# HongwenZhang/DaNet-DensePose2SMPL

Hardware: AMD Instinct MI355X
Metric: images/sec fwd+bwd HRNet-W48+SMPL+IUV 256x256 bs32/GPU (higher is better)
Workload: dtype bf16; 1 GPU; full DaNet train step (HRNet-W48 + global and part-wise IUV heads + regressor nets + SMPL LBS (2 forward + 1 backward; the 2 label-side forwards belong to the untimed batch prologue) + IUV render + losses, fwd+bwd+Adam), 256x256, 32 img/GPU; convs bf16 MFMA fp32-acc, LBS/raster/losses fp32; global_batch=32, parallelism=dp1

## Files before the change

### danet-densepose2smpl_amd/_lib.py

```python
import ctypes
import os

_HERE = os.path.dirname(os.path.abspath(__file__))
LIB_PATH = os.environ.get('DANET_LIB') or os.path.join(_HERE, 'csrc', 'libdanet_hip.so')
_lib = None

c_f = ctypes.c_void_p
c_i = ctypes.c_int
c_sz = ctypes.c_size_t
c_fl = ctypes.c_float

_SIGNATURES = {
    'danet_version': (c_i, []),
    'danet_last_error': (ctypes.c_char_p, []),
    'danet_smpl_lbs_debug': (c_i, [c_f]),
    'danet_smpl_lbs_ctx_floats': (c_sz, [c_i]),
    'danet_smpl_lbs_fwd_ws_floats': (c_sz, [c_i, c_i, c_i]),
    'danet_smpl_lbs_bwd_ws_floats': (c_sz, [c_i, c_i, c_i]),
    'danet_smpl_lbs_ticket_words': (c_sz, [c_i]),
    'danet_smpl_lbs_forward': (c_i, [c_f, c_f, c_i] + [c_f] * 9 + [c_i] * 4 + [c_f] * 5 + [c_sz, c_f, c_f]),
    'danet_smpl_lbs_backward': (c_i, [c_f, c_f, c_i] + [c_f] * 7 + [c_i] * 4 + [c_f] * 7 + [c_sz, c_f, c_i, c_f]),
    'danet_smpl_lbs_backward_fused_ok': (c_i, [c_i, c_i, c_i]),
    'danet_iuv_raster_ws_bytes': (c_sz, [c_i, c_i, c_i]),
    'danet_iuv_raster_forward': (c_i, [c_f, c_f, c_i, c_i, c_f, c_i, c_f, c_f, c_i, c_fl, c_fl, c_i, c_f, c_f, c_f, c_f, c_sz, c_f]),
# ... 13 lines not shown
    'danet_conv_f32m_forward': (c_i, [c_f, c_f, c_f, c_f] + [c_i] * 15 + [c_f]),
    'danet_conv_f32m_wgrad_ws_floats': (c_sz, [c_i] * 15),
    'danet_conv_f32m_wgrad': (c_i, [c_f, c_f, c_f, c_f] + [c_i] * 15 + [c_f]),
    'danet_conv3x3_debug': (None, [c_f]),
    'danet_conv3x3_stream_plan': (c_i, [c_i] * 6),
    'danet_conv_stem_ok': (c_i, [c_i] * 13),
    'danet_conv_stem_forward': (c_i, [c_f, c_f, c_f] + [c_i] * 7 + [c_f, c_f]),
    'danet_conv_stem_dgrad_ok': (c_i, [c_i] * 13),
    'danet_conv_stem_dgrad': (c_i, [c_f, c_f, c_f] + [c_i] * 7 + [c_f] * 5),
    'danet_conv3x3a_ok': (c_i, [c_i] * 11),
    'danet_conv3x3a': (c_i, [c_f, c_f, c_f] + [c_i] * 4 + [c_f] * 5 + [c_i, c_f, c_f]),
    'danet_conv3x3_stream_table_bytes': (c_sz, []),
    'danet_conv3x3_stream_tables': (c_i, [c_f, c_sz]),
    'danet_conv_pack_weights_batched': (c_i, [c_f, c_i, ctypes.c_long, ctypes.c_long, c_f]),
    'danet_conv_pack_job_bricks': (ctypes.c_long, [c_i] * 7),
    'danet_conv_forward_multi_ok': (c_i, [c_f, c_i]),
    'danet_conv_forward_multi_kernel': (c_i, [c_f, c_i]),
    'danet_conv_forward_multi': (c_i, [c_f, c_i, c_f]),
    'danet_conv_forward_multi_epi_ok': (c_i, [c_f, c_i]),
    'danet_conv_forward_multi_epi_kernel': (c_i, [c_f, c_i]),
    'danet_conv_forward_multi_epi': (c_i, [c_f, c_i, c_f]),
    'danet_conv_stem_forward_epi': (c_i, [c_f, c_f, c_f, c_f] + [c_i] * 8 + [c_f]),
    'danet_conv3x3a_forward_epi': (c_i, [c_f] * 5 + [c_i] * 4 + [c_f]),
    'danet_conv_bn_forward_multi_ok': (c_i, [c_f, c_i, c_f, c_f]),
    'danet_conv_bn_forward_multi': (c_i, [c_f, c_i, c_f, c_fl, c_fl, c_f, c_f, c_f]),
    'danet_conv_forward_kernel': (c_i, [c_i] * 15),
    'danet_conv_forward': (c_i, [c_f] * 4 + [c_i] * 16 + [c_f] * 6 + [c_i, c_f]),
    'danet_conv_wgrad_rows_ok': (c_i, [c_i] * 13),
    'danet_conv_wgrad_rows_ws_floats': (c_sz, [c_i] * 8),
    'danet_conv_wgrad_rows': (c_i, [c_f] * 4 + [c_sz] + [c_i] * 12 + [c_fl, c_f]),
    'danet_conv_wgrad3x3_ok': (c_i, [c_i] * 10),
    'danet_conv_wgrad3x3_pair_ok': (c_i, [c_i] * 11),
    'danet_conv_wgrad3x3_ws_floats': (c_sz, [c_i] * 7),
    'danet_conv_wgrad_multi_ws_floats': (c_sz, [c_f, c_i]),
    'danet_conv_wgrad_multi_ws_zero_from': (c_sz, [c_f, c_i]),
    'danet_conv_wgrad_multi': (c_i, [c_f, c_i, c_f, c_sz, c_fl, c_f]),
    'danet_conv_wgrad3x3_multi_ws_floats': (c_sz, [c_f, c_i]),
    'danet_conv_wgrad3x3_multi': (c_i, [c_f, c_i, c_f, c_sz, c_fl, c_f]),
    'danet_conv_wgrad3x3_kernel_id': (c_i, [c_i] * 7),
    'danet_conv_wgrad3x3': (c_i, [c_f] * 4 + [c_sz] + [c_i] * 7 + [c_fl, c_i, c_f]),
    'danet_conv_wgrad_ws_floats': (c_sz, [c_i] * 4),
    'danet_conv_wgrad_ws_floats_for': (c_sz, [c_i] * 13),
    'danet_conv_wgrad': (c_i, [c_f] * 4 + [c_sz] + [c_i] * 13 + [c_fl, c_i, c_f]),
    'danet_bn_forward': (c_i, [c_f, c_f, c_f, ctypes.c_int64, c_i] + [c_f] * 6 + [c_i, c_fl, c_fl, c_i, c_i, c_f, c_f]),
    'danet_bn_ws_floats': (c_sz, [c_i]),
    'danet_knob': (ctypes.c_long, [c_i, ctypes.c_long]),
    'danet_bn_acc_bytes': (c_i, []),
    'danet_channel_sum': (c_i, [c_f, ctypes.c_int64, c_i, c_f, c_i, c_i, c_f]),
    'danet_bn_forward_multi': (c_i, [c_f, c_i, c_fl, c_fl, c_f]),
    'danet_bn_backward_multi': (c_i, [c_f, c_i, c_f]),
    'danet_bn_backward_onepass_ok': (c_i, [c_f, c_i, c_i]),
    'danet_bn_backward_onepass_bar_words': (c_i, []),
    'danet_bn_backward_onepass': (c_i, [c_f, c_i, c_f, c_i, c_f]),
    'danet_bn_backward': (c_i, [c_f, c_f, c_f, ctypes.c_int64, c_i, c_f, c_f, c_i, c_f, c_f, c_f, c_f, c_i, c_i, c_f, c_f, c_f]),
    'danet_sum_relu_forward': (c_i, [ctypes.POINTER(ctypes.c_void_p), ctypes.POINTER(c_i), c_i, c_i, c_i, c_i, c_i, c_i, c_f, c_f]),
    'danet_sum_relu_backward': (c_i, [c_f, c_f, c_i, c_i, c_i, c_i, c_i, c_i, c_f, c_f]),
    'danet_sum_relu_backward_all': (c_i, [c_f, c_f] + [c_i] * 5 + [c_f] * 5),
    'danet_sum_relu_forward_multi': (c_i, [c_f, c_i, c_f]),
    'danet_sum_relu_backward_all_multi': (c_i, [c_f, c_i, c_f]),
    'danet_maxpool3x3s2_forward': (c_i, [c_f, c_f, c_f, c_i, c_i, c_i, c_i, c_f]),
    'danet_maxpool3x3s2_backward': (c_i, [c_f, c_f, c_f, c_i, c_i, c_i, c_i, c_f]),
    'danet_stn_gather_forward': (c_i, [c_f, c_f] + [c_i] * 8 + [c_f, c_f]),
    'danet_stn_gather_backward': (c_i, [c_f, c_f] + [c_i] * 8 + [c_f, c_f]),
    'danet_part_clean_forward': (c_i, [c_f, c_f, c_i, c_i, c_i, c_i, c_f, c_f]),
    'danet_part_clean_backward': (c_i, [c_f, c_f, c_f, c_i, c_i, c_i, c_i, c_f, c_f]),
    'danet_part_loss_forward': (c_i, [c_f] * 5 + [c_i] * 5 + [c_f, c_f]),
# ... 219 lines not shown
```

### danet-densepose2smpl_amd/csrc/conv_wgrad3x3.hip

```cpp
#include <cstdlib>
#include "common.h"
#include "conv_common.h"

namespace {

using namespace danet_conv;

constexpr int TH = 4, TW = 8;
constexpr int halo_h(int st) { return st * (TH - 1) + 3; }
constexpr int halo_w(int st) { return st * (TW - 1) + 3; }

struct Wg3P {
    const bf16_t* x; const bf16_t* dy; float* part;
    float* direct;
    int B, H, W, Cin, Cout, groups, Cin_g, Cout_g;
    int IH, IW;
    int tiles_h, tiles_w, msplit;
    long nchunks;
    long x_bytes, dy_bytes;
};

typedef __attribute__((ext_vector_type(2))) unsigned v2u;

__device__ inline v2u tr_read(unsigned lds_byte_addr) {
    v2u r;
    asm volatile("ds_read_b64_tr_b16 %0, %1" : "=v"(r) : "v"(lds_byte_addr) : "memory");
    return r;
}

template <int CT, int NI, int ST, int SM = 0>
__device__ __forceinline__ void wgrad3x3_body(const Wg3P& p, const int bx, const int by, const int bz)
{
    constexpr bool PAIR = SM != 0;
    constexpr int OS = SM ? SM : 4;
    constexpr int PHW = ST * (OS - 1) + 3;
    constexpr int IMH = SM ? TH / OS : 1, IMW = SM ? TW / OS : 1;
    constexpr int HH = SM ? IMH * PHW : halo_h(ST), HW = SM ? IMW * PHW : halo_w(ST);
    constexpr int HALF = SM ? (4 / OS) * PHW : ST * 4;
    constexpr int BCO = CT * 16, BCI = NI * 16;
    constexpr int PXY = BCO * 2, PXX = BCI * 2;
    extern __shared__ __attribute__((aligned(16))) unsigned char smem[];
    constexpr int YB = TH * TW * PXY, XB = HH * HW * PXX, BUF = YB + XB;

    const int t = threadIdx.x, lane = t & 63, wave = t >> 6;
    const int li = lane & 15, lg = lane >> 4;
    const int nci = (p.Cin_g + BCI - 1) / BCI;
    const int cib = by % nci, cob = by / nci;
    const int g = bz;
    const int co0 = cob * BCO, ci0 = cib * BCI;
    const bf16_t* const dyg = p.dy + (size_t)g * p.Cout_g + co0;
    const bf16_t* const xg = p.x + (size_t)g * p.Cin_g + ci0;

    constexpr int NPAIR = 9 * NI;
    constexpr int MAXP = (NPAIR + 3) / 4;
    f32x4 acc[MAXP][CT];
    unsigned boff[MAXP];
#pragma unroll
    for (int pi = 0; pi < MAXP; ++pi) {
#pragma unroll
        for (int ct = 0; ct < CT; ++ct) acc[pi][ct] = f32x4{0.f, 0.f, 0.f, 0.f};
        const int pair = min(wave + 4 * pi, NPAIR - 1);
        const int tap = pair / NI, ni = pair - tap * NI;
        const int r = tap / 3, s = tap - r * 3;
        const int hrow = SM ? (lg / OS) * PHW + ST * (lg % OS) + r : ST * lg + r;
        const int hcol = SM ? ((li >> 2) / OS) * PHW + ST * ((li >> 2) % OS) + s : ST * (li >> 2) + s;
        boff[pi] = (unsigned)((hrow * HW + hcol) * PXX + (ni * 16 + 4 * (li & 3)) * 2);
    }
    const unsigned aoff = (unsigned)((lg * TW + (li >> 2)) * PXY + (4 * (li & 3)) * 2);

    const int nchunks = (int)p.nchunks;
    const int per = (nchunks + p.msplit - 1) / p.msplit;
    const int c_begin = bx * per, c_end = min(nchunks, c_begin + per);

    constexpr int NPY = TH * TW * (BCO / 8), NPX = HH * HW * (BCI / 8);
    constexpr int NRY = (NPY + 255) / 256, NRX = (NPX + 255) / 256;
    constexpr int OOB = 0x7fffffff;
    const __amdgpu_buffer_rsrc_t yr = __builtin_amdgcn_make_buffer_rsrc(const_cast<bf16_t*>(dyg), 0, (int)p.dy_bytes, 0x00020000);
    const __amdgpu_buffer_rsrc_t xr = __builtin_amdgcn_make_buffer_rsrc(const_cast<bf16_t*>(xg), 0, (int)p.x_bytes, 0x00020000);
    int yrel[NRY], xrel[NRX], xhy[NRX], xhx[NRX];
#pragma unroll
    for (int u = 0; u < NRY; ++u) {
        const int pc = t + u * 256;
        const int c8 = pc % (BCO / 8), q = pc / (BCO / 8);
        const int ty = q / TW, tx = q % TW;
        const int ypix = SM ? ((ty / OS) * IMW + tx / OS) * (OS * OS) + (ty % OS) * OS + tx % OS : ty * p.W + tx;
        yrel[u] = (pc < NPY && co0 + c8 * 8 < p.Cout_g) ? (ypix * p.Cout + c8 * 8) * 2 : OOB;
    }
#pragma unroll
    for (int u = 0; u < NRX; ++u) {
        const int pc = t + u * 256;
        const int c8 = pc % (BCI / 8), q = pc / (BCI / 8);
        const bool live = pc < NPX && ci0 + c8 * 8 < p.Cin_g;
        if (PAIR) {
            const int hq = q / HW, img = (hq / PHW) * IMW + (q % HW) / PHW, hy = hq % PHW - 1, hc = (q % HW) % PHW - 1;
            const bool inside = live && (unsigned)hy < (unsigned)(OS * ST) && (unsigned)hc < (unsigned)(OS * ST);
            xrel[u] = ((img * (OS * OS * ST * ST) + hy * (OS * ST) + hc) * p.Cin + c8 * 8) * 2;
            xhy[u] = inside ? 1 : -100000;
            xhx[u] = 1;
        } else {
            xrel[u] = (((q / HW - 1) * p.IW + q % HW - 1) * p.Cin + c8 * 8) * 2;
            xhy[u] = live ? q / HW : -100000;
            xhx[u] = q % HW;
        }
    }
    int f_tw = c_begin % p.tiles_w, f_th = (c_begin / p.tiles_w) % p.tiles_h, f_b = c_begin / (p.tiles_w * p.tiles_h);
    uint4 ystage[NRY], xstage[NRX];

    auto fetch = [&]() {
        const int oh0 = f_th * TH, ow0 = f_tw * TW;
        const int pix0 = (f_b * p.H + oh0) * p.W + ow0;
        const int by = pix0 * p.Cout * 2, bx = ((f_b * p.IH + ST * oh0) * p.IW + ST * ow0) * p.Cin * 2;
#pragma unroll
        for (int u = 0; u < NRY; ++u)
            ystage[u] = __builtin_bit_cast(uint4, __builtin_amdgcn_raw_buffer_load_b128(yr, yrel[u] != OOB ? by + yrel[u] : OOB, 0, 0));
#pragma unroll
        for (int u = 0; u < NRX; ++u) {
            const bool ok = PAIR ? xhy[u] > 0
                                 : ((unsigned)(ST * oh0 - 1 + xhy[u]) < (unsigned)p.IH && (unsigned)(ST * ow0 - 1 + xhx[u]) < (unsigned)p.IW);
            xstage[u] = __builtin_bit_cast(uint4, __builtin_amdgcn_raw_buffer_load_b128(xr, ok ? bx + xrel[u] : OOB, 0, 0));
        }
        if (++f_tw == p.tiles_w) { f_tw = 0; if (++f_th == p.tiles_h) { f_th = 0; ++f_b; } }
    };
    auto commit = [&](int buf) {
        unsigned char* base = smem + buf * BUF;
#pragma unroll
        for (int u = 0; u < NRY; ++u)
            if (t + u * 256 < NPY) *reinterpret_cast<uint4*>(base + (size_t)(t + u * 256) * 16) = ystage[u];
#pragma unroll
        for (int u = 0; u < NRX; ++u)
            if (t + u * 256 < NPX) *reinterpret_cast<uint4*>(base + (size_t)(NPY + t + u * 256) * 16) = xstage[u];
    };

    if (c_begin < c_end) fetch();
    int buf = 0;
    for (int ch = c_begin; ch < c_end; ++ch) {
        commit(buf);
        __syncthreads();
        if (ch + 1 < c_end) fetch();
        const unsigned ybase = (unsigned)(buf * BUF), xbase = ybase + YB;
        v2u alo[CT], ahi[CT], blo[MAXP], bhi[MAXP];
#pragma unroll
        for (int ct = 0; ct < CT; ++ct) {
            alo[ct] = tr_read(ybase + aoff + ct * 32);
            ahi[ct] = tr_read(ybase + aoff + ct * 32 + 4 * PXY);
        }
#pragma unroll
        for (int pi = 0; pi < MAXP; ++pi) {
            blo[pi] = tr_read(xbase + boff[pi]);
            bhi[pi] = tr_read(xbase + boff[pi] + HALF * PXX);
        }
        asm volatile("s_waitcnt lgkmcnt(0)" ::: "memory");
        __builtin_amdgcn_sched_barrier(0);
        bf16x8 a[CT];
#pragma unroll
        for (int ct = 0; ct < CT; ++ct) {
            const uint4 raw = {alo[ct].x, alo[ct].y, ahi[ct].x, ahi[ct].y};
            a[ct] = __builtin_bit_cast(bf16x8, raw);
        }
#pragma unroll
        for (int pi = 0; pi < MAXP; ++pi) {
            const uint4 raw = {blo[pi].x, blo[pi].y, bhi[pi].x, bhi[pi].y};
            const bf16x8 bq = __builtin_bit_cast(bf16x8, raw);
#pragma unroll
            for (int ct = 0; ct < CT; ++ct)
                acc[pi][ct] = __builtin_amdgcn_mfma_f32_16x16x32_bf16(a[ct], bq, acc[pi][ct], 0, 0, 0);
        }
        buf ^= 1;
    }
    const int gsz = 9 * p.Cout_g * p.Cin_g;
    if (p.direct) {
        float* const dw = p.direct + (size_t)g * gsz;
#pragma unroll
        for (int pi = 0; pi < MAXP; ++pi) {
            const int pair = wave + 4 * pi;
            const int tap = pair / NI, ni = pair - tap * NI;
            const int cin = ci0 + ni * 16 + li;
            if (pair >= NPAIR || cin >= p.Cin_g) continue;
#pragma unroll
            for (int ct = 0; ct < CT; ++ct)
#pragma unroll
                for (int r = 0; r < 4; ++r) {
                    const int cout = co0 + ct * 16 + lg * 4 + r;
                    if (cout < p.Cout_g) dw[((size_t)cout * p.Cin_g + cin) * 9 + tap] = acc[pi][ct][r];
                }
        }
        return;
    }
    float* dst = p.part + ((size_t)bx * p.groups + g) * gsz;
#pragma unroll
    for (int pi = 0; pi < MAXP; ++pi) {
        const int pair = wave + 4 * pi;
        const int tap = pair / NI, ni = pair - tap * NI;
        const int cin = ci0 + ni * 16 + li;
        if (pair >= NPAIR || cin >= p.Cin_g) continue;
        float* row = dst + ((tap * p.Cout_g + co0 + lg * 4) * p.Cin_g + cin);
#pragma unroll
        for (int ct = 0; ct < CT; ++ct)
#pragma unroll
            for (int r = 0; r < 4; ++r)
                if (co0 + ct * 16 + lg * 4 + r < p.Cout_g) row[(ct * 16 + r) * p.Cin_g] = acc[pi][ct][r];
    }
}

template <int CT, int NI, int ST>
__global__ __launch_bounds__(256) void conv_wgrad3x3_kernel(Wg3P p)
{
    wgrad3x3_body<CT, NI, ST>(p, blockIdx.x, blockIdx.y, blockIdx.z);
}

constexpr int NPM = 20;
struct Wg3Multi { Wg3P p[NPM]; int start[NPM + 1]; int nyb[NPM]; int n; int xcd; };

template <int CT, int NI, int ST, int SM = 0>
__global__ __launch_bounds__(256) void conv_wgrad3x3_multi_kernel(Wg3Multi mp)
{
    int vb = (int)blockIdx.x;
    if (mp.xcd) {
        const int G = (int)gridDim.x, q = G >> 3, r = G & 7;
        const int x = vb & 7, slot = vb >> 3;
        vb = x * q + (x < r ? x : r) + slot;
    }
    int i = 0;
    while (i + 1 < mp.n && vb >= mp.start[i + 1]) ++i;
    const int l = vb - mp.start[i];
    const Wg3P& p = mp.p[i];
    const int bx = l % p.msplit, rest = l / p.msplit;
    wgrad3x3_body<CT, NI, ST, SM>(p, bx, rest % mp.nyb[i], rest / mp.nyb[i]);
}

struct Red3Multi { const float* part[NPM]; float* dw[NPM]; int G[NPM], Cout_g[NPM], Cin_g[NPM], msplit[NPM]; long start[NPM + 1]; int n; float beta; };

__global__ __launch_bounds__(256) void wgrad3x3_reduce_multi_kernel(Red3Multi rp)
{
    const long gidx = (long)blockIdx.x * 256 + threadIdx.x;
    if (gidx >= rp.start[rp.n]) return;
    int i = 0;
    while (i + 1 < rp.n && gidx >= rp.start[i + 1]) ++i;
    const long idx = gidx - rp.start[i], total = rp.start[i + 1] - rp.start[i];
    const float* part = rp.part[i];
    float s = 0.f;
    int sp = 0;
    for (; sp + 4 <= rp.msplit[i]; sp += 4) {
        const float v0 = part[(size_t)sp * total + idx], v1 = part[(size_t)(sp + 1) * total + idx];
        const float v2 = part[(size_t)(sp + 2) * total + idx], v3 = part[(size_t)(sp + 3) * total + idx];
        s += (v0 + v1) + (v2 + v3);
    }
    for (; sp < rp.msplit[i]; ++sp) s += part[(size_t)sp * total + idx];
    const int Cin_g = rp.Cin_g[i], Cout_g = rp.Cout_g[i];
    const int cin = (int)(idx % Cin_g);
    long rest = idx / Cin_g;
    const int cout = (int)(rest % Cout_g); rest /= Cout_g;
    const int tap = (int)(rest % 9), g = (int)(rest / 9);
    const size_t o = (((size_t)(g * Cout_g + cout)) * Cin_g + cin) * 9 + tap;
    float* dw = rp.dw[i];
    dw[o] = rp.beta != 0.f ? dw[o] * rp.beta + s : s;
}

__global__ __launch_bounds__(256) void wgrad3x3_reduce_kernel(const float* __restrict__ part, float* __restrict__ dw,
                                                               int G, int Cout_g, int Cin_g, int msplit, float beta)
{
    const long total = (long)G * Cout_g * Cin_g * 9;
    const long idx = (long)blockIdx.x * 256 + threadIdx.x;
    if (idx >= total) return;
    float s = 0.f;
    int sp = 0;
    for (; sp + 4 <= msplit; sp += 4) {
        const float v0 = part[(size_t)sp * total + idx], v1 = part[(size_t)(sp + 1) * total + idx];
        const float v2 = part[(size_t)(sp + 2) * total + idx], v3 = part[(size_t)(sp + 3) * total + idx];
        s += (v0 + v1) + (v2 + v3);
    }
    for (; sp < msplit; ++sp) s += part[(size_t)sp * total + idx];
    const int cin = (int)(idx % Cin_g);
    long rest = idx / Cin_g;
    const int cout = (int)(rest % Cout_g); rest /= Cout_g;
    const int tap = (int)(rest % 9), g = (int)(rest / 9);
    const size_t o = (((size_t)(g * Cout_g + cout)) * Cin_g + cin) * 9 + tap;
    dw[o] = beta != 0.f ? dw[o] * beta + s : s;
}

template <int CT, int NI, int ST>
int launch3(const Wg3P& p, hipStream_t st) {
    const int nco = (p.Cout_g + CT * 16 - 1) / (CT * 16), nci = (p.Cin_g + NI * 16 - 1) / (NI * 16);
    const size_t lds = 2 * (size_t)(TH * TW * CT * 32 + halo_h(ST) * halo_w(ST) * NI * 32);
    hipLaunchKernelGGL((conv_wgrad3x3_kernel<CT, NI, ST>), dim3(p.msplit, nco * nci, p.groups), dim3(256), lds, st, p);
    return 0;
}

inline int tiles3(int c) { return c <= 16 ? 1 : (c <= 32 ? 2 : ((c % 48 == 0 || c <= 48) ? 3 : 4)); }

}

extern "C" int danet_conv_wgrad3x3_ok(int H, int W, int Cin, int Cout, int R, int S, int stride, int pad, int dil, int groups) {
    static const bool no_s2 = getenv("DANET_NO_WGRAD3_S2") != nullptr;
    if (!(R == 3 && S == 3 && (stride == 1 || (stride == 2 && !no_s2)) && pad == 1 && dil == 1)) return 0;
    if (H % stride != 0 || W % stride != 0) return 0;
    return (H / stride) % TH == 0 && (W / stride) % TW == 0 && (Cin / groups) % 8 == 0 && (Cout / groups) % 8 == 0;
}

extern "C" int danet_conv_wgrad3x3_pair_ok(int B, int H, int W, int Cin, int Cout, int R, int S, int stride, int pad, int dil, int groups) {
    static const bool off = getenv("DANET_NO_WGRAD3_PAIR") != nullptr;
    if (off || !(R == 3 && S == 3 && (stride == 1 || stride == 2) && pad == 1 && dil == 1 && H == W && B > 0 && groups > 0)) return 0;
    if (!((H == 4 * stride && B % 2 == 0) || (H == 2 * stride && B % 8 == 0))) return 0;
    if (Cin % groups != 0 || Cout % groups != 0) return 0;
    const int ci = Cin / groups, co = Cout / groups;
    if (ci % 8 != 0 || co % 8 != 0) return 0;
    return 1;
}
static inline int wg3_small(int B, int H, int W, int stride) {
    if (!(stride == 1 || stride == 2) || H != W) return 0;
    if (H == 4 * stride && B % 2 == 0) return 4;
    if (H == 2 * stride && B % 8 == 0) return 2;
    return 0;
}
static inline bool wg3_is_pair(int B, int H, int W, int stride) { return wg3_small(B, H, W, stride) != 0; }

static void plan3(int B, int H, int W, int Cin, int Cout, int groups, int* ct, int* ni, int* msplit) {
    const int Cout_g = Cout / groups, Cin_g = Cin / groups;
    *ct = tiles3(Cout_g); *ni = tiles3(Cin_g);
    if (*ct == 4) *ct = 2;
    if (*ni == 4) *ni = 2;
    const long other = (long)((Cout_g + *ct * 16 - 1) / (*ct * 16)) * ((Cin_g + *ni * 16 - 1) / (*ni * 16)) * groups;
    const long nchunks = (long)B * (H / TH) * (W / TW);
    long target = 256;
    if (const char* e = getenv("DANET_WGRAD3_BLOCKS")) target = atol(e);
    long ms = (target + other - 1) / other;
    if (ms > nchunks / 4) ms = nchunks / 4;
    if (ms < 1) ms = 1;
    *msplit = (int)ms;
}

extern "C" int danet_conv_wgrad3x3_kernel_id(int B, int H, int W, int Cin, int Cout, int groups, int stride) {
    int ct, ni, ms;
    plan3(B, H / stride, W / stride, Cin, Cout, groups, &ct, &ni, &ms);
    return ct * 10 + ni;
}

extern "C" size_t danet_conv_wgrad3x3_ws_floats(int B, int H, int W, int Cin, int Cout, int groups, int stride) {
    int ct, ni, ms;
    if (stride < 1) return 0;
    plan3(B, H / stride, W / stride, Cin, Cout, groups, &ct, &ni, &ms);
    return (size_t)ms * Cout * (Cin / groups) * 9;
}

extern "C" int danet_conv_wgrad3x3(const void* x, const void* dy, float* dw, float* ws, size_t ws_floats,
                                   int B, int H, int W, int Cin, int Cout, int groups, int stride, float beta, int phase, void* stream)
{
    DANET_ENTER();
    DANET_CHECK_ARG(x && dy && dw && ws && B > 0 && phase >= 0 && phase <= 2, "conv_wgrad3x3: bad arguments");
    DANET_CHECK_ARG(danet_conv_wgrad3x3_ok(H, W, Cin, Cout, 3, 3, stride, 1, 1, groups), "conv_wgrad3x3: unsupported shape");
    Wg3P p;
    p.x = (const bf16_t*)x; p.dy = (const bf16_t*)dy; p.part = ws; p.direct = nullptr;
    p.IH = H; p.IW = W; H /= stride; W /= stride;
    p.B = B; p.H = H; p.W = W; p.Cin = Cin; p.Cout = Cout; p.groups = groups;
    p.Cin_g = Cin / groups; p.Cout_g = Cout / groups;
    p.tiles_h = H / TH; p.tiles_w = W / TW;
    p.nchunks = (long)B * p.tiles_h * p.tiles_w;
    p.x_bytes = (long)B * p.IH * p.IW * Cin * 2; p.dy_bytes = (long)B * H * W * Cout * 2;
    DANET_CHECK_ARG(p.x_bytes < (1L << 31) && p.dy_bytes < (1L << 31), "conv_wgrad3x3: tensors of 2 GB or more are not supported");
    int ct, ni;
    plan3(B, H, W, Cin, Cout, groups, &ct, &ni, &p.msplit);
    if (ws_floats < (size_t)p.msplit * Cout * p.Cin_g * 9)
        return danet::fail(DANET_ERR_WORKSPACE, "conv_wgrad3x3: workspace too small");
    hipStream_t st = (hipStream_t)stream;
    if (phase != 2) {
#define W3(a, b) if (ct == a && ni == b) { if (stride == 1) launch3<a, b, 1>(p, st); else launch3<a, b, 2>(p, st); } else
        W3(1, 1) W3(1, 2) W3(1, 3) W3(2, 1) W3(2, 2) W3(2, 3) W3(3, 1) W3(3, 2) W3(3, 3)
        return danet::fail(DANET_ERR_ARG, "conv_wgrad3x3: no kernel for tiles %dx%d", ct, ni);
#undef W3
        DANET_CHECK_LAUNCH("conv_wgrad3x3_kernel");
    }
    if (phase == 1) return DANET_OK;
    const long total = (long)Cout * p.Cin_g * 9;
    hipLaunchKernelGGL(wgrad3x3_reduce_kernel, dim3(danet::cdiv(total, 256)), dim3(256), 0, st, ws, dw, groups, p.Cout_g,
                       p.Cin_g, p.msplit, beta);
    DANET_CHECK_LAUNCH("wgrad3x3_reduce_kernel");
    return DANET_OK;
}


struct Wg3Job { const void* x; const void* dy; float* dw; int B, H, W, Cin, Cout, groups, stride; };

static long multi_target_blocks() {
    if (const char* e = getenv("DANET_WGRAD3_MULTI_BLOCKS")) return atol(e);
    return 768;
}

static inline double wg3_weight(int Cout, int Cin_g) { const double p = (double)Cout * Cin_g; return p < 2304.0 ? 2304.0 : p; }
static void plan_multi(const Wg3Job* jobs, const int* idx, int cnt, int ct, int ni, int* msplit) {
    auto chunks_of = [](const Wg3Job& j) -> long {
        const int sm = wg3_small(j.B, j.H, j.W, j.stride);
        return sm ? (long)(j.B / (sm == 4 ? 2 : 8)) : (long)j.B * (j.H / j.stride / TH) * (j.W / j.stride / TW);
    };
    double tot = 0;
    for (int k = 0; k < cnt; ++k) {
        const Wg3Job& j = jobs[idx[k]];
        tot += (double)chunks_of(j) * wg3_weight(j.Cout, j.Cin / j.groups);
    }
    const long target = multi_target_blocks();
    for (int k = 0; k < cnt; ++k) {
        const Wg3Job& j = jobs[idx[k]];
        const int Cout_g = j.Cout / j.groups, Cin_g = j.Cin / j.groups;
        const long other = (long)((Cout_g + ct * 16 - 1) / (ct * 16)) * ((Cin_g + ni * 16 - 1) / (ni * 16)) * j.groups;
        const long nchunks = chunks_of(j);
        const double w = (double)nchunks * wg3_weight(j.Cout, Cin_g);
        long ms = (long)(target * (w / tot) / other + 0.5);
        if (ms > nchunks / 4) ms = nchunks / 4;
        if (ms < 1) ms = 1;
        msplit[k] = (int)ms;
    }
}

static int multi_foreach_launch(const Wg3Job* jobs, int n, float* ws, size_t ws_floats, float beta, hipStream_t st, size_t* need_out)
{
    size_t used = 0;
    bool done[4096];
    if (n > 4096) return danet::fail(DANET_ERR_ARG, "conv_wgrad3x3_multi: too many jobs (%d)", n);
    for (int i = 0; i < n; ++i) done[i] = false;
    for (int i = 0; i < n; ++i) {
        if (done[i]) continue;
        int ct, ni, dummy;
        const int stride = jobs[i].stride;
        const int sm = wg3_small(jobs[i].B, jobs[i].H, jobs[i].W, stride);
        const bool pair = sm != 0;
        plan3(jobs[i].B, jobs[i].H / stride, jobs[i].W / stride, jobs[i].Cin, jobs[i].Cout, jobs[i].groups, &ct, &ni, &dummy);
        static const int npm_env = getenv("DANET_WGRAD3_NPM") ? atoi(getenv("DANET_WGRAD3_NPM")) : 0;
        const int npm = npm_env > 0 && npm_env < NPM ? npm_env : NPM;
        int idx[NPM], cnt = 0;
        for (int k = i; k < n && cnt < npm; ++k) {
            if (done[k] || jobs[k].stride != stride || wg3_small(jobs[k].B, jobs[k].H, jobs[k].W, stride) != sm) continue;
            int c2, n2;
            plan3(jobs[k].B, jobs[k].H / stride, jobs[k].W / stride, jobs[k].Cin, jobs[k].Cout, jobs[k].groups, &c2, &n2, &dummy);
            if (c2 == ct && n2 == ni) { idx[cnt++] = k; done[k] = true; }
        }
        int msplit[NPM];
        plan_multi(jobs, idx, cnt, ct, ni, msplit);
        Wg3Multi mp; Red3Multi rp;
        static const bool xcd_order = getenv("DANET_WGRAD3_XCD") && atoi(getenv("DANET_WGRAD3_XCD")) != 0;
        mp.n = cnt; rp.n = cnt; rp.beta = beta; mp.xcd = xcd_order ? 1 : 0;
        mp.start[0] = 0; rp.start[0] = 0;
        for (int k = 0; k < cnt; ++k) {
            const Wg3Job& j = jobs[idx[k]];
            Wg3P& p = mp.p[k];
            static const bool no_direct = getenv("DANET_WGRAD3_NO_DIRECT") != nullptr;
            const bool direct = msplit[k] == 1 && beta == 0.f && !no_direct;
            p.x = (const bf16_t*)j.x; p.dy = (const bf16_t*)j.dy; p.part = (ws && !direct) ? ws + used : nullptr;
            p.direct = direct ? j.dw : nullptr;
            p.IH = j.H; p.IW = j.W;
            p.B = j.B; p.H = j.H / stride; p.W = j.W / stride; p.Cin = j.Cin; p.Cout = j.Cout; p.groups = j.groups;
            if (pair) { p.B = j.B / (sm == 4 ? 2 : 8); p.H = 4; p.W = 8; p.IH = 4 * stride; p.IW = 8 * stride; }
            p.Cin_g = j.Cin / j.groups; p.Cout_g = j.Cout / j.groups;
            p.tiles_h = p.H / TH; p.tiles_w = p.W / TW;
            p.nchunks = (long)p.B * p.tiles_h * p.tiles_w;
            p.x_bytes = (long)j.B * j.H * j.W * j.Cin * 2; p.dy_bytes = (long)j.B * (j.H / stride) * (j.W / stride) * j.Cout * 2;
            p.msplit = msplit[k];
            const int nyb = ((p.Cout_g + ct * 16 - 1) / (ct * 16)) * ((p.Cin_g + ni * 16 - 1) / (ni * 16));
            mp.nyb[k] = nyb;
            mp.start[k + 1] = mp.start[k] + msplit[k] * nyb * j.groups;
            const long total = (long)j.Cout * p.Cin_g * 9;
            rp.part[k] = p.part; rp.dw[k] = j.dw; rp.G[k] = j.groups; rp.Cout_g[k] = p.Cout_g; rp.Cin_g[k] = p.Cin_g; rp.msplit[k] = msplit[k];
            rp.start[k + 1] = rp.start[k] + (direct ? 0 : total);
            if (!direct || !ws) used += (size_t)msplit[k] * total;
            if (ws && !(p.x_bytes < (1L << 31) && p.dy_bytes < (1L << 31)))
                return danet::fail(DANET_ERR_ARG, "conv_wgrad3x3_multi: tensors of 2 GB or more are not supported");
        }
        if (!ws) continue;
        if (used > ws_floats) return danet::fail(DANET_ERR_WORKSPACE, "conv_wgrad3x3_multi: workspace too small");
        const int phw = stride * ((sm ? sm : 4) - 1) + 3;
        const size_t lds = 2 * (size_t)(TH * TW * ct * 32 + (sm ? (TH / sm) * phw * (TW / sm) * phw : halo_h(stride) * halo_w(stride)) * ni * 32);
        const dim3 grid((unsigned)mp.start[cnt]);
        if (pair) {
#define W3P(a, b) if (ct == a && ni == b) { \
            if (stride == 1 && sm == 4) hipLaunchKernelGGL((conv_wgrad3x3_multi_kernel<a, b, 1, 4>), grid, dim3(256), lds, st, mp); \
            else if (stride == 2 && sm == 4) hipLaunchKernelGGL((conv_wgrad3x3_multi_kernel<a, b, 2, 4>), grid, dim3(256), lds, st, mp); \
            else if (stride == 1) hipLaunchKernelGGL((conv_wgrad3x3_multi_kernel<a, b, 1, 2>), grid, dim3(256), lds, st, mp); \
            else hipLaunchKernelGGL((conv_wgrad3x3_multi_kernel<a, b, 2, 2>), grid, dim3(256), lds, st, mp); } else
            W3P(2, 2) W3P(2, 3) W3P(3, 2) W3P(3, 3) W3P(1, 1) W3P(1, 2) W3P(2, 1) W3P(1, 3) W3P(3, 1)
            return danet::fail(DANET_ERR_ARG, "conv_wgrad3x3_multi: no pair-mode kernel for tiles %dx%d", ct, ni);
#undef W3P
        } else
#define W3M(a, b) if (ct == a && ni == b) { \
            if (stride == 1) hipLaunchKernelGGL((conv_wgrad3x3_multi_kernel<a, b, 1>), grid, dim3(256), lds, st, mp); \
            else hipLaunchKernelGGL((conv_wgrad3x3_multi_kernel<a, b, 2>), grid, dim3(256), lds, st, mp); } else
        W3M(1, 1) W3M(1, 2) W3M(1, 3) W3M(2, 1) W3M(2, 2) W3M(2, 3) W3M(3, 1) W3M(3, 2) W3M(3, 3)
        return danet::fail(DANET_ERR_ARG, "conv_wgrad3x3_multi: no kernel for tiles %dx%d", ct, ni);
#undef W3M
        DANET_CHECK_LAUNCH("conv_wgrad3x3_multi_kernel");
        if (rp.start[cnt] > 0) {
            hipLaunchKernelGGL(wgrad3x3_reduce_multi_kernel, dim3((unsigned)danet::cdiv(rp.start[cnt], 256)), dim3(256), 0, st, rp);
            DANET_CHECK_LAUNCH("wgrad3x3_reduce_multi_kernel");
        }
    }
    if (need_out) *need_out = used;
    return DANET_OK;
}

extern "C" size_t danet_conv_wgrad3x3_multi_ws_floats(const void* jobs, int n)
{
    size_t need = 0;
    if (!jobs || n <= 0) return 0;
    multi_foreach_launch((const Wg3Job*)jobs, n, nullptr, 0, 0.f, nullptr, &need);
    return need;
}

// ... 13 lines not shown
```

### include/danet_hip.h

```cpp
#ifndef DANET_HIP_H
#define DANET_HIP_H

#include <stddef.h>
#include <stdint.h>

#ifdef __cplusplus
extern "C" {
#endif

#define DANET_OK 0
#define DANET_ERR_ARG (-1)
#define DANET_ERR_HIP (-2)
#define DANET_ERR_WORKSPACE (-3)

int danet_version(void);
const char* danet_last_error(void);

size_t danet_smpl_lbs_ctx_floats(int B);
size_t danet_smpl_lbs_fwd_ws_floats(int B, int V, int NE);
size_t danet_smpl_lbs_bwd_ws_floats(int B, int V, int NB);
size_t danet_smpl_lbs_ticket_words(int B);

int danet_smpl_lbs_forward(const float* betas, const float* rotmats, int B,
                           const float* v_template, const float* shapedirs, const float* posedirs,
// ... 161 lines not shown
       DANET_KNOB_PW = 10, DANET_KNOB_PW_WGRAD = 11, DANET_KNOB_STEM = 12, DANET_KNOB_STEM_DGRAD = 13, DANET_KNOB_C3A = 14,
       DANET_KNOB_BN_BLOCK_BYTES = 15, DANET_KNOB_C3S_BALANCE = 16, DANET_KNOB_C3S_TILE_COST = 17,
       DANET_KNOB_G3 = 18  };
long danet_knob(int id, long value);
int danet_conv3x3_stream_plan(int B, int H, int W, int Cin, int Cout, int nprob);
size_t danet_conv3x3_stream_table_bytes(void);
int danet_conv3x3_stream_tables(void* workspace, size_t bytes);
int danet_conv_stem_ok(int B, int H, int W, int Cin, int OH, int OW, int Cout, int R, int S, int stride, int pad, int dil, int groups);
int danet_conv_stem_forward(const void* x, const void* wp, void* y, int B, int H, int W, int Cin, int OH, int OW, int Cout,
                            float* bn_sums, void* stream);
int danet_conv_stem_forward_epi(const void* x, const void* wp, const float* bias, void* y, int B, int H, int W, int Cin, int OH, int OW,
                                int Cout, int relu, void* stream);
int danet_conv_stem_dgrad_ok(int B, int H, int W, int Cin, int OH, int OW, int Cout, int R, int S, int stride, int pad, int dil, int groups);
int danet_conv_stem_dgrad(const void* dy, const void* wp, void* dx, int B, int H, int W, int Cin, int OH, int OW, int Cout,
                          const void* bn_x, const void* bn_y, const float* bn_saved, float* bn_red, void* stream);
int danet_conv3x3a_ok(int B, int H, int W, int Cin, int Cout, int R, int S, int stride, int pad, int dil, int groups);
int danet_conv3x3a(const void* x, const void* wp, void* y, int B, int H, int W, int transposed, float* bn_sums,
                   const void* bn_x, const void* bn_y, const float* bn_saved, float* bn_red, int bn_gate, const void* addend, void* stream);
int danet_conv3x3a_forward_epi(const void* x, const void* wp, const float* bias, const void* addend, void* y, int B, int H, int W,
                               int relu, void* stream);
void danet_conv3x3_debug(int* dev_buf);
int danet_conv_forward_multi(const void* jobs, int n, void* stream);
int danet_conv_forward_kernel(int B, int H, int W, int Cin, int OH, int OW, int Cout, int R, int S,
                              int stride, int pad, int dil, int groups, int transposed, int out_fp32);
int danet_conv_forward(const void* x, const void* wp, const float* bias, void* y,
                       int B, int H, int W, int Cin, int OH, int OW, int Cout,
                       int R, int S, int stride, int pad, int dil, int groups, int transposed,
                       int relu, int out_fp32, float* bn_sums,
                       const void* bn_x, const void* bn_y, const float* bn_saved, float* bn_red, const void* addend,
                       int bn_gate, void* stream);
int danet_conv_wgrad3x3_ok(int H, int W, int Cin, int Cout, int R, int S, int stride, int pad, int dil, int groups);
int danet_conv_wgrad3x3_pair_ok(int B, int H, int W, int Cin, int Cout, int R, int S, int stride, int pad, int dil, int groups);
size_t danet_conv_wgrad3x3_ws_floats(int B, int H, int W, int Cin, int Cout, int groups, int stride);
size_t danet_conv_wgrad3x3_multi_ws_floats(const void* jobs, int n);
size_t danet_conv_wgrad_multi_ws_floats(const void* jobs, int n);
size_t danet_conv_wgrad_multi_ws_zero_from(const void* jobs, int n);
int danet_conv_wgrad_multi(const void* jobs, int n, float* ws, size_t ws_floats, float beta, void* stream);
int danet_conv_wgrad3x3_multi(const void* jobs, int n, float* ws, size_t ws_floats, float beta, void* stream);
int danet_conv_wgrad3x3_kernel_id(int B, int H, int W, int Cin, int Cout, int groups, int stride);
int danet_conv_wgrad3x3(const void* x, const void* dy, float* dw, float* ws, size_t ws_floats,
                        int B, int H, int W, int Cin, int Cout, int groups, int stride, float beta, int phase , void* stream);
int danet_conv_wgrad_rows_ok(int B, int H, int W, int Cin, int OH, int OW, int Cout, int R, int S, int stride, int pad, int dil, int groups);
size_t danet_conv_wgrad_rows_ws_floats(int B, int OH, int OW, int Cin, int Cout, int R, int S, int groups);
int danet_conv_wgrad_rows(const void* x, const void* dy, float* dw, float* ws, size_t ws_floats,
                          int B, int H, int W, int Cin, int OH, int OW, int Cout,
                          int R, int S, int stride, int pad, int groups, float beta, void* stream);
size_t danet_conv_wgrad_ws_floats(int Cout, int Cin_g, int R, int S);
size_t danet_conv_wgrad_ws_floats_for(int B, int H, int W, int Cin, int OH, int OW, int Cout, int R, int S, int stride, int pad, int dil, int groups);
int danet_conv_wgrad(const void* x, const void* dy, float* dw, float* ws, size_t ws_floats,
                     int B, int H, int W, int Cin, int OH, int OW, int Cout,
                     int R, int S, int stride, int pad, int dil, int groups, float beta, int ws_is_zero, void* stream);

int danet_bn_forward(const void* x, const void* res, void* y, int64_t M, int C,
                     const float* gamma, const float* beta, float* running_mean, float* running_var,
                     float* saved, float* sums_ws, int ws_is_zero, float momentum, float eps, int training, int relu,
                     void* relu_mask, void* stream);
size_t danet_bn_ws_floats(int C);
int danet_bn_acc_bytes(void);
int danet_bn_backward(const void* dy, const void* x, const void* y, int64_t M, int C,
                      const float* gamma, const float* saved, int relu,
                      void* dx, void* dres, float* dparam, float* red_ws, int ws_is_zero,
                      int mask_mode, const void* relu_mask, const float* beta, void* stream);
int danet_bn_forward_multi(const void* jobs, int n, float momentum, float eps, void* stream);
int danet_bn_backward_multi(const void* jobs, int n, void* stream);
int danet_bn_backward_onepass_bar_words(void);
int danet_bn_backward_onepass_ok(const void* jobs, int n, int max_blocks);
// ... 62 lines not shown
```

Baseline: 1356 images/sec.

## Add 8x16 super-chunk wgrad3x3 path with LDS-direct DMA double buffering

Adds a super-chunk variant of the 3x3 weight-gradient kernel for stride-1 maps divisible by 8x16. Each chunk covers an 8x16 output tile, so the halo overhead per output pixel shrinks. Tiles are loaded straight into LDS with buffer_load...lds, double-buffered, and the LDS transposed reads are software-pipelined across four sub-tiles. Block targets, msplit caps and the multi-job grouping are adjusted for the larger chunks, and the XCD block-reordering option is removed. The trade-off is more LDS per block (launch bounds set to 2 blocks per CU) and fewer chunks to split across blocks.

```diff
diff --git a/danet-densepose2smpl_amd/_lib.py b/danet-densepose2smpl_amd/_lib.py
--- a/danet-densepose2smpl_amd/_lib.py
+++ b/danet-densepose2smpl_amd/_lib.py
@@ -69,6 +69,7 @@
     'danet_conv_wgrad3x3_ok': (c_i, [c_i] * 10),
     'danet_conv_wgrad3x3_pair_ok': (c_i, [c_i] * 11),
     'danet_conv_wgrad3x3_ws_floats': (c_sz, [c_i] * 7),
+    'danet_conv_wgrad3x3_chunk_mode': (c_i, [c_i] * 4),
     'danet_conv_wgrad_multi_ws_floats': (c_sz, [c_f, c_i]),
     'danet_conv_wgrad_multi_ws_zero_from': (c_sz, [c_f, c_i]),
     'danet_conv_wgrad_multi': (c_i, [c_f, c_i, c_f, c_sz, c_fl, c_f]),
diff --git a/danet-densepose2smpl_amd/csrc/conv_wgrad3x3.hip b/danet-densepose2smpl_amd/csrc/conv_wgrad3x3.hip
--- a/danet-densepose2smpl_amd/csrc/conv_wgrad3x3.hip
+++ b/danet-densepose2smpl_amd/csrc/conv_wgrad3x3.hip
@@ -9,6 +9,8 @@
 constexpr int TH = 4, TW = 8;
 constexpr int halo_h(int st) { return st * (TH - 1) + 3; }
 constexpr int halo_w(int st) { return st * (TW - 1) + 3; }
+constexpr int SCH = 8, SCW = 16;
+typedef __attribute__((address_space(3))) void* lds_ptr_t;
 
 struct Wg3P {
     const bf16_t* x; const bf16_t* dy; float* part;
@@ -27,20 +29,26 @@
     asm volatile("ds_read_b64_tr_b16 %0, %1" : "=v"(r) : "v"(lds_byte_addr) : "memory");
     return r;
 }
-
-template <int CT, int NI, int ST, int SM = 0>
+__device__ __forceinline__ void dma16(unsigned lds_addr, int voff, const __amdgpu_buffer_rsrc_t& desc) {
+    asm volatile("s_mov_b32 m0, %0\n\ts_nop 0\n\tbuffer_load_dwordx4 %1, %2, 0 offen lds" :: "s"(lds_addr), "v"(voff), "s"(desc) : "memory");
+}
+
+template <int CT, int NI, int ST, int SM = 0, int SC = 0>
 __device__ __forceinline__ void wgrad3x3_body(const Wg3P& p, const int bx, const int by, const int bz)
 {
     constexpr bool PAIR = SM != 0;
     constexpr int OS = SM ? SM : 4;
     constexpr int PHW = ST * (OS - 1) + 3;
     constexpr int IMH = SM ? TH / OS : 1, IMW = SM ? TW / OS : 1;
-    constexpr int HH = SM ? IMH * PHW : halo_h(ST), HW = SM ? IMW * PHW : halo_w(ST);
+    static_assert(!SC || (SM == 0 && ST == 1), "super-chunks: stride 1, ordinary maps");
+    constexpr int CH = SC ? SCH : TH, CW = SC ? SCW : TW;
+    constexpr int NK = CH * CW / 32;
+    constexpr int HH = SM ? IMH * PHW : ST * (CH - 1) + 3, HW = SM ? IMW * PHW : ST * (CW - 1) + 3;
     constexpr int HALF = SM ? (4 / OS) * PHW : ST * 4;
     constexpr int BCO = CT * 16, BCI = NI * 16;
     constexpr int PXY = BCO * 2, PXX = BCI * 2;
     extern __shared__ __attribute__((aligned(16))) unsigned char smem[];
-    constexpr int YB = TH * TW * PXY, XB = HH * HW * PXX, BUF = YB + XB;
+    constexpr int YB = CH * CW * PXY, XB = HH * HW * PXX, BUF = YB + XB;
 
     const int t = threadIdx.x, lane = t & 63, wave = t >> 6;
     const int li = lane & 15, lg = lane >> 4;
@@ -66,13 +74,13 @@
         const int hcol = SM ? ((li >> 2) / OS) * PHW + ST * ((li >> 2) % OS) + s : ST * (li >> 2) + s;
         boff[pi] = (unsigned)((hrow * HW + hcol) * PXX + (ni * 16 + 4 * (li & 3)) * 2);
     }
-    const unsigned aoff = (unsigned)((lg * TW + (li >> 2)) * PXY + (4 * (li & 3)) * 2);
+    const unsigned aoff = (unsigned)((lg * CW + (li >> 2)) * PXY + (4 * (li & 3)) * 2);
 
     const int nchunks = (int)p.nchunks;
     const int per = (nchunks + p.msplit - 1) / p.msplit;
     const int c_begin = bx * per, c_end = min(nchunks, c_begin + per);
 
-    constexpr int NPY = TH * TW * (BCO / 8), NPX = HH * HW * (BCI / 8);
+    constexpr int NPY = CH * CW * (BCO / 8), NPX = HH * HW * (BCI / 8);
     constexpr int NRY = (NPY + 255) / 256, NRX = (NPX + 255) / 256;
     constexpr int OOB = 0x7fffffff;
     const __amdgpu_buffer_rsrc_t yr = __builtin_amdgcn_make_buffer_rsrc(const_cast<bf16_t*>(dyg), 0, (int)p.dy_bytes, 0x00020000);
@@ -82,7 +90,7 @@
     for (int u = 0; u < NRY; ++u) {
         const int pc = t + u * 256;
         const int c8 = pc % (BCO / 8), q = pc / (BCO / 8);
-        const int ty = q / TW, tx = q % TW;
+        const int ty = q / CW, tx = q % CW;
         const int ypix = SM ? ((ty / OS) * IMW + tx / OS) * (OS * OS) + (ty % OS) * OS + tx % OS : ty * p.W + tx;
         yrel[u] = (pc < NPY && co0 + c8 * 8 < p.Cout_g) ? (ypix * p.Cout + c8 * 8) * 2 : OOB;
     }
@@ -104,6 +112,68 @@
         }
     }
     int f_tw = c_begin % p.tiles_w, f_th = (c_begin / p.tiles_w) % p.tiles_h, f_b = c_begin / (p.tiles_w * p.tiles_h);
+    if constexpr (SC) {
+        const unsigned lds0 = (unsigned)(unsigned long long)(lds_ptr_t)smem + (unsigned)(wave * 1024);
+        auto issue = [&](int buf) {
+            const int oh0 = f_th * CH, ow0 = f_tw * CW;
+            const int by = ((f_b * p.H + oh0) * p.W + ow0) * p.Cout * 2, bx = ((f_b * p.IH + oh0) * p.IW + ow0) * p.Cin * 2;
+            const unsigned dst = __builtin_amdgcn_readfirstlane(lds0 + (unsigned)(buf * BUF));
+#pragma unroll
+            for (int u = 0; u < NRY; ++u)
+                dma16(dst + u * 4096, yrel[u] != OOB ? by + yrel[u] : OOB, yr);
+#pragma unroll
+            for (int u = 0; u < NRX; ++u) {
+                const bool ok = (unsigned)(oh0 - 1 + xhy[u]) < (unsigned)p.IH && (unsigned)(ow0 - 1 + xhx[u]) < (unsigned)p.IW;
+                if (t + u * 256 < NPX) dma16(dst + YB + u * 4096, ok ? bx + xrel[u] : OOB, xr);
+            }
+            if (++f_tw == p.tiles_w) { f_tw = 0; if (++f_th == p.tiles_h) { f_th = 0; ++f_b; } }
+        };
+        if (c_begin < c_end) issue(0);
+        int buf = 0;
+        for (int ch = c_begin; ch < c_end; ++ch) {
+            asm volatile("s_waitcnt vmcnt(0)" ::: "memory");
+            __syncthreads();
+            if (ch + 1 < c_end) issue(buf ^ 1);
+            const unsigned ybase = (unsigned)(buf * BUF), xbase = ybase + YB;
+            v2u alo[2][CT], ahi[2][CT], blo[2][MAXP], bhi[2][MAXP];
+            auto rd = [&](int k) {
+                const unsigned ya = ybase + aoff + (unsigned)(((k >> 1) * TH * CW + (k & 1) * TW) * PXY);
+                const unsigned xa = xbase + (unsigned)(((k >> 1) * TH * HW + (k & 1) * TW) * PXX);
+#pragma unroll
+                for (int ct = 0; ct < CT; ++ct) {
+                    alo[k & 1][ct] = tr_read(ya + ct * 32);
+                    ahi[k & 1][ct] = tr_read(ya + ct * 32 + 4 * PXY);
+                }
+#pragma unroll
+                for (int pi = 0; pi < MAXP; ++pi) {
+                    blo[k & 1][pi] = tr_read(xa + boff[pi]);
+                    bhi[k & 1][pi] = tr_read(xa + boff[pi] + HALF * PXX);
+                }
+            };
+            rd(0);
+#pragma unroll
+            for (int k = 0; k < NK; ++k) {
+                asm volatile("s_waitcnt lgkmcnt(0)" ::: "memory");
+                __builtin_amdgcn_sched_barrier(0);
+                if (k + 1 < NK) { rd(k + 1); __builtin_amdgcn_sched_barrier(0); }
+                bf16x8 a[CT];
+#pragma unroll
+                for (int ct = 0; ct < CT; ++ct) {
+                    const uint4 raw = {alo[k & 1][ct].x, alo[k & 1][ct].y, ahi[k & 1][ct].x, ahi[k & 1][ct].y};
+                    a[ct] = __builtin_bit_cast(bf16x8, raw);
+                }
+#pragma unroll
+                for (int pi = 0; pi < MAXP; ++pi) {
+                    const uint4 raw = {blo[k & 1][pi].x, blo[k & 1][pi].y, bhi[k & 1][pi].x, bhi[k & 1][pi].y};
+                    const bf16x8 bq = __builtin_bit_cast(bf16x8, raw);
+#pragma unroll
+                    for (int ct = 0; ct < CT; ++ct)
+                        acc[pi][ct] = __builtin_amdgcn_mfma_f32_16x16x32_bf16(a[ct], bq, acc[pi][ct], 0, 0, 0);
+                }
+            }
+            buf ^= 1;
+        }
+    } else {
     uint4 ystage[NRY], xstage[NRX];
 
     auto fetch = [&]() {
@@ -167,6 +237,7 @@
         }
         buf ^= 1;
     }
+    }
     const int gsz = 9 * p.Cout_g * p.Cin_g;
     if (p.direct) {
         float* const dw = p.direct + (size_t)g * gsz;
@@ -207,25 +278,36 @@
 {
     wgrad3x3_body<CT, NI, ST>(p, blockIdx.x, blockIdx.y, blockIdx.z);
 }
+template <int CT, int NI>
+__global__ __launch_bounds__(256, 2) void conv_wgrad3x3_sc_kernel(Wg3P p)
+{
+    wgrad3x3_body<CT, NI, 1, 0, 1>(p, blockIdx.x, blockIdx.y, blockIdx.z);
+}
 
 constexpr int NPM = 20;
-struct Wg3Multi { Wg3P p[NPM]; int start[NPM + 1]; int nyb[NPM]; int n; int xcd; };
-
-template <int CT, int NI, int ST, int SM = 0>
-__global__ __launch_bounds__(256) void conv_wgrad3x3_multi_kernel(Wg3Multi mp)
-{
-    int vb = (int)blockIdx.x;
-    if (mp.xcd) {
-        const int G = (int)gridDim.x, q = G >> 3, r = G & 7;
-        const int x = vb & 7, slot = vb >> 3;
-        vb = x * q + (x < r ? x : r) + slot;
-    }
+struct Wg3Multi { Wg3P p[NPM]; int start[NPM + 1]; int nyb[NPM]; int n; };
+
+template <int CT, int NI, int ST, int SM, int SC>
+__device__ __forceinline__ void wgrad3x3_multi_body(const Wg3Multi& mp)
+{
+    const int vb = (int)blockIdx.x;
     int i = 0;
     while (i + 1 < mp.n && vb >= mp.start[i + 1]) ++i;
     const int l = vb - mp.start[i];
     const Wg3P& p = mp.p[i];
     const int bx = l % p.msplit, rest = l / p.msplit;
-    wgrad3x3_body<CT, NI, ST, SM>(p, bx, rest % mp.nyb[i], rest / mp.nyb[i]);
+    wgrad3x3_body<CT, NI, ST, SM, SC>(p, bx, rest % mp.nyb[i], rest / mp.nyb[i]);
+}
+
+template <int CT, int NI, int ST, int SM = 0>
+__global__ __launch_bounds__(256) void conv_wgrad3x3_multi_kernel(Wg3Multi mp)
+{
+    wgrad3x3_multi_body<CT, NI, ST, SM, 0>(mp);
+}
+template <int CT, int NI>
+__global__ __launch_bounds__(256, 2) void conv_wgrad3x3_multi_sc_kernel(Wg3Multi mp)
+{
+    wgrad3x3_multi_body<CT, NI, 1, 0, 1>(mp);
 }
 
 struct Red3Multi { const float* part[NPM]; float* dw[NPM]; int G[NPM], Cout_g[NPM], Cin_g[NPM], msplit[NPM]; long start[NPM + 1]; int n; float beta; };
@@ -285,6 +367,13 @@
     hipLaunchKernelGGL((conv_wgrad3x3_kernel<CT, NI, ST>), dim3(p.msplit, nco * nci, p.groups), dim3(256), lds, st, p);
     return 0;
 }
+constexpr size_t sc_lds(int ct, int ni) { return 2 * (size_t)(SCH * SCW * ct * 32 + (SCH + 2) * (SCW + 2) * ni * 32); }
+template <int CT, int NI>
+int launch3_sc(const Wg3P& p, hipStream_t st) {
+    const int nco = (p.Cout_g + CT * 16 - 1) / (CT * 16), nci = (p.Cin_g + NI * 16 - 1) / (NI * 16);
+    hipLaunchKernelGGL((conv_wgrad3x3_sc_kernel<CT, NI>), dim3(p.msplit, nco * nci, p.groups), dim3(256), sc_lds(CT, NI), st, p);
+    return 0;
+}
 
 inline int tiles3(int c) { return c <= 16 ? 1 : (c <= 32 ? 2 : ((c % 48 == 0 || c <= 48) ? 3 : 4)); }
 
@@ -313,32 +402,38 @@
     return 0;
 }
 static inline bool wg3_is_pair(int B, int H, int W, int stride) { return wg3_small(B, H, W, stride) != 0; }
-
-static void plan3(int B, int H, int W, int Cin, int Cout, int groups, int* ct, int* ni, int* msplit) {
+static inline bool wg3_super(int H, int W, int stride) { return stride == 1 && H % SCH == 0 && W % SCW == 0; }
+extern "C" int danet_conv_wgrad3x3_chunk_mode(int B, int H, int W, int stride) {
+    if (wg3_small(B, H, W, stride)) return 2;
+    return wg3_super(H, W, stride) ? 1 : 0;
+}
+
+static void plan3(int B, int H, int W, int Cin, int Cout, int groups, int* ct, int* ni, int* msplit, bool sc = false) {
     const int Cout_g = Cout / groups, Cin_g = Cin / groups;
     *ct = tiles3(Cout_g); *ni = tiles3(Cin_g);
     if (*ct == 4) *ct = 2;
     if (*ni == 4) *ni = 2;
     const long other = (long)((Cout_g + *ct * 16 - 1) / (*ct * 16)) * ((Cin_g + *ni * 16 - 1) / (*ni * 16)) * groups;
-    const long nchunks = (long)B * (H / TH) * (W / TW);
+    const long nchunks = sc ? (long)B * (H / SCH) * (W / SCW) : (long)B * (H / TH) * (W / TW);
     long target = 256;
     if (const char* e = getenv("DANET_WGRAD3_BLOCKS")) target = atol(e);
     long ms = (target + other - 1) / other;
-    if (ms > nchunks / 4) ms = nchunks / 4;
+    const long cap = sc ? nchunks / 2 : nchunks / 4;
+    if (ms > cap) ms = cap;
     if (ms < 1) ms = 1;
     *msplit = (int)ms;
 }
 
 extern "C" int danet_conv_wgrad3x3_kernel_id(int B, int H, int W, int Cin, int Cout, int groups, int stride) {
     int ct, ni, ms;
-    plan3(B, H / stride, W / stride, Cin, Cout, groups, &ct, &ni, &ms);
+    plan3(B, H / stride, W / stride, Cin, Cout, groups, &ct, &ni, &ms, wg3_super(H, W, stride));
     return ct * 10 + ni;
 }
 
 extern "C" size_t danet_conv_wgrad3x3_ws_floats(int B, int H, int W, int Cin, int Cout, int groups, int stride) {
     int ct, ni, ms;
     if (stride < 1) return 0;
-    plan3(B, H / stride, W / stride, Cin, Cout, groups, &ct, &ni, &ms);
+    plan3(B, H / stride, W / stride, Cin, Cout, groups, &ct, &ni, &ms, wg3_super(H, W, stride));
     return (size_t)ms * Cout * (Cin / groups) * 9;
 }
 
@@ -350,20 +445,21 @@
     DANET_CHECK_ARG(danet_conv_wgrad3x3_ok(H, W, Cin, Cout, 3, 3, stride, 1, 1, groups), "conv_wgrad3x3: unsupported shape");
     Wg3P p;
     p.x = (const bf16_t*)x; p.dy = (const bf16_t*)dy; p.part = ws; p.direct = nullptr;
+    const bool sc = wg3_super(H, W, stride);
     p.IH = H; p.IW = W; H /= stride; W /= stride;
     p.B = B; p.H = H; p.W = W; p.Cin = Cin; p.Cout = Cout; p.groups = groups;
     p.Cin_g = Cin / groups; p.Cout_g = Cout / groups;
-    p.tiles_h = H / TH; p.tiles_w = W / TW;
+    p.tiles_h = H / (sc ? SCH : TH); p.tiles_w = W / (sc ? SCW : TW);
     p.nchunks = (long)B * p.tiles_h * p.tiles_w;
     p.x_bytes = (long)B * p.IH * p.IW * Cin * 2; p.dy_bytes = (long)B * H * W * Cout * 2;
     DANET_CHECK_ARG(p.x_bytes < (1L << 31) && p.dy_bytes < (1L << 31), "conv_wgrad3x3: tensors of 2 GB or more are not supported");
     int ct, ni;
-    plan3(B, H, W, Cin, Cout, groups, &ct, &ni, &p.msplit);
+    plan3(B, H, W, Cin, Cout, groups, &ct, &ni, &p.msplit, sc);
     if (ws_floats < (size_t)p.msplit * Cout * p.Cin_g * 9)
         return danet::fail(DANET_ERR_WORKSPACE, "conv_wgrad3x3: workspace too small");
     hipStream_t st = (hipStream_t)stream;
     if (phase != 2) {
-#define W3(a, b) if (ct == a && ni == b) { if (stride == 1) launch3<a, b, 1>(p, st); else launch3<a, b, 2>(p, st); } else
+#define W3(a, b) if (ct == a && ni == b) { if (sc) launch3_sc<a, b>(p, st); else if (stride == 1) launch3<a, b, 1>(p, st); else launch3<a, b, 2>(p, st); } else
         W3(1, 1) W3(1, 2) W3(1, 3) W3(2, 1) W3(2, 2) W3(2, 3) W3(3, 1) W3(3, 2) W3(3, 3)
         return danet::fail(DANET_ERR_ARG, "conv_wgrad3x3: no kernel for tiles %dx%d", ct, ni);
 #undef W3
@@ -380,15 +476,16 @@
 
 struct Wg3Job { const void* x; const void* dy; float* dw; int B, H, W, Cin, Cout, groups, stride; };
 
-static long multi_target_blocks() {
+static long multi_target_blocks(bool sc) {
     if (const char* e = getenv("DANET_WGRAD3_MULTI_BLOCKS")) return atol(e);
-    return 768;
+    return sc ? 480 : 768;
 }
 
 static inline double wg3_weight(int Cout, int Cin_g) { const double p = (double)Cout * Cin_g; return p < 2304.0 ? 2304.0 : p; }
-static void plan_multi(const Wg3Job* jobs, const int* idx, int cnt, int ct, int ni, int* msplit) {
-    auto chunks_of = [](const Wg3Job& j) -> long {
+static void plan_multi(const Wg3Job* jobs, const int* idx, int cnt, int ct, int ni, bool sc, int* msplit) {
+    auto chunks_of = [sc](const Wg3Job& j) -> long {
         const int sm = wg3_small(j.B, j.H, j.W, j.stride);
+        if (sc) return (long)j.B * (j.H / SCH) * (j.W / SCW);
         return sm ? (long)(j.B / (sm == 4 ? 2 : 8)) : (long)j.B * (j.H / j.stride / TH) * (j.W / j.stride / TW);
     };
     double tot = 0;
@@ -396,7 +493,7 @@
         const Wg3Job& j = jobs[idx[k]];
         tot += (double)chunks_of(j) * wg3_weight(j.Cout, j.Cin / j.groups);
     }
-    const long target = multi_target_blocks();
+    const long target = multi_target_blocks(sc);
     for (int k = 0; k < cnt; ++k) {
         const Wg3Job& j = jobs[idx[k]];
         const int Cout_g = j.Cout / j.groups, Cin_g = j.Cin / j.groups;
@@ -404,7 +501,8 @@
         const long nchunks = chunks_of(j);
         const double w = (double)nchunks * wg3_weight(j.Cout, Cin_g);
         long ms = (long)(target * (w / tot) / other + 0.5);
-        if (ms > nchunks / 4) ms = nchunks / 4;
+        const long cap = sc ? nchunks / 2 : nchunks / 4;
+        if (ms > cap) ms = cap;
         if (ms < 1) ms = 1;
         msplit[k] = (int)ms;
     }
@@ -422,21 +520,22 @@
         const int stride = jobs[i].stride;
         const int sm = wg3_small(jobs[i].B, jobs[i].H, jobs[i].W, stride);
         const bool pair = sm != 0;
+        const bool sc = !pair && wg3_super(jobs[i].H, jobs[i].W, stride);
         plan3(jobs[i].B, jobs[i].H / stride, jobs[i].W / stride, jobs[i].Cin, jobs[i].Cout, jobs[i].groups, &ct, &ni, &dummy);
         static const int npm_env = getenv("DANET_WGRAD3_NPM") ? atoi(getenv("DANET_WGRAD3_NPM")) : 0;
         const int npm = npm_env > 0 && npm_env < NPM ? npm_env : NPM;
         int idx[NPM], cnt = 0;
         for (int k = i; k < n && cnt < npm; ++k) {
             if (done[k] || jobs[k].stride != stride || wg3_small(jobs[k].B, jobs[k].H, jobs[k].W, stride) != sm) continue;
+            if ((!pair && wg3_super(jobs[k].H, jobs[k].W, stride)) != sc) continue;
             int c2, n2;
             plan3(jobs[k].B, jobs[k].H / stride, jobs[k].W / stride, jobs[k].Cin, jobs[k].Cout, jobs[k].groups, &c2, &n2, &dummy);
             if (c2 == ct && n2 == ni) { idx[cnt++] = k; done[k] = true; }
         }
         int msplit[NPM];
-        plan_multi(jobs, idx, cnt, ct, ni, msplit);
+        plan_multi(jobs, idx, cnt, ct, ni, sc, msplit);
         Wg3Multi mp; Red3Multi rp;
-        static const bool xcd_order = getenv("DANET_WGRAD3_XCD") && atoi(getenv("DANET_WGRAD3_XCD")) != 0;
-        mp.n = cnt; rp.n = cnt; rp.beta = beta; mp.xcd = xcd_order ? 1 : 0;
+        mp.n = cnt; rp.n = cnt; rp.beta = beta;
         mp.start[0] = 0; rp.start[0] = 0;
         for (int k = 0; k < cnt; ++k) {
             const Wg3Job& j = jobs[idx[k]];
@@ -449,7 +548,7 @@
             p.B = j.B; p.H = j.H / stride; p.W = j.W / stride; p.Cin = j.Cin; p.Cout = j.Cout; p.groups = j.groups;
             if (pair) { p.B = j.B / (sm == 4 ? 2 : 8); p.H = 4; p.W = 8; p.IH = 4 * stride; p.IW = 8 * stride; }
             p.Cin_g = j.Cin / j.groups; p.Cout_g = j.Cout / j.groups;
-            p.tiles_h = p.H / TH; p.tiles_w = p.W / TW;
+            p.tiles_h = p.H / (sc ? SCH : TH); p.tiles_w = p.W / (sc ? SCW : TW);
             p.nchunks = (long)p.B * p.tiles_h * p.tiles_w;
             p.x_bytes = (long)j.B * j.H * j.W * j.Cin * 2; p.dy_bytes = (long)j.B * (j.H / stride) * (j.W / stride) * j.Cout * 2;
             p.msplit = msplit[k];
@@ -468,7 +567,12 @@
         const int phw = stride * ((sm ? sm : 4) - 1) + 3;
         const size_t lds = 2 * (size_t)(TH * TW * ct * 32 + (sm ? (TH / sm) * phw * (TW / sm) * phw : halo_h(stride) * halo_w(stride)) * ni * 32);
         const dim3 grid((unsigned)mp.start[cnt]);
-        if (pair) {
+        if (sc) {
+#define W3S(a, b) if (ct == a && ni == b) hipLaunchKernelGGL((conv_wgrad3x3_multi_sc_kernel<a, b>), grid, dim3(256), sc_lds(a, b), st, mp); else
+            W3S(1, 1) W3S(1, 2) W3S(1, 3) W3S(2, 1) W3S(2, 2) W3S(2, 3) W3S(3, 1) W3S(3, 2) W3S(3, 3)
+            return danet::fail(DANET_ERR_ARG, "conv_wgrad3x3_multi: no super-chunk kernel for tiles %dx%d", ct, ni);
+#undef W3S
+        } else if (pair) {
 #define W3P(a, b) if (ct == a && ni == b) { \
             if (stride == 1 && sm == 4) hipLaunchKernelGGL((conv_wgrad3x3_multi_kernel<a, b, 1, 4>), grid, dim3(256), lds, st, mp); \
             else if (stride == 2 && sm == 4) hipLaunchKernelGGL((conv_wgrad3x3_multi_kernel<a, b, 2, 4>), grid, dim3(256), lds, st, mp); \
diff --git a/include/danet_hip.h b/include/danet_hip.h
--- a/include/danet_hip.h
+++ b/include/danet_hip.h
@@ -217,6 +217,7 @@
 int danet_conv_wgrad3x3_ok(int H, int W, int Cin, int Cout, int R, int S, int stride, int pad, int dil, int groups);
 int danet_conv_wgrad3x3_pair_ok(int B, int H, int W, int Cin, int Cout, int R, int S, int stride, int pad, int dil, int groups);
 size_t danet_conv_wgrad3x3_ws_floats(int B, int H, int W, int Cin, int Cout, int groups, int stride);
+int danet_conv_wgrad3x3_chunk_mode(int B, int H, int W, int stride);
 size_t danet_conv_wgrad3x3_multi_ws_floats(const void* jobs, int n);
 size_t danet_conv_wgrad_multi_ws_floats(const void* jobs, int n);
 size_t danet_conv_wgrad_multi_ws_zero_from(const void* jobs, int n);
```

Result: no change. 1362 images/sec (median of 6 runs) (+0.4%).
